# raviraina/grok

Measured on AMD Instinct MI355X. Metric: Mpixels/s encode+decode, 8K RGB 5/3 lossless + 9/7 lossy, 1/2/4/8 GPU, higher is better.
Workload: dtype int32 (5/3) + f32 (9/7)

## Files before the change

### grok_amd/csrc/gk_engine.cpp

```cpp
#include <hip/hip_runtime.h>

#include <algorithm>
#include <array>
#include <tuple>
#include <cmath>
#include <cstdarg>
#include <cstdlib>
#include <cstdio>
#include <cstring>
#include <memory>
#include <string>
#include <atomic>
#include <chrono>
#include <condition_variable>
#include <functional>
#include <mutex>
#include <thread>
#include <unordered_map>
#include <vector>
#include <queue>
#include <map>
#include <climits>
#include <linux/futex.h>
#include <sys/syscall.h>
// ... 2892 lines not shown
    bool dwt_partial = false;
    uint32_t dec_reduce = 0;
    bool win_whole_tile = false;
    int device = 0;
    bool registered = false;
    hipStream_t st = nullptr;
    hipStream_t aux[3] = {nullptr, nullptr, nullptr};
    hipEvent_t xev[6];
    std::string err;
    gk_timings tm{};
    std::string plan_key;
    Plan plan;
    DevBuf arena;
    DevBuf bytes;
    DevBuf dblocks;
    DevBuf dpasses;
    DevBuf dinfo;
    DevBuf dseg;
    DevBuf dout;
    DevBuf dplanes;
    DevBuf derr;
    DevBuf dsym, dsymoff, dpassend, dcminfo;
    DevBuf dmsstate, dseglen;
    DevBuf dscratch, dnmse, dord, dweight, dord_enc;
    HostBuf hinfo, hseg, hhdr, hpasses, hord, hweight, hord_enc;
    DevBuf dstage1, dstage2;
    DevBuf dcol_src, dcol_out, dcol_tab;
    DevBuf dpix_src, dpix_out;
    DevBuf dicc_tab;
    std::vector<uint8_t> icc_blob;
    DevBuf dpix_in;
    HostBuf hstage1, hstage2;
    int16_t* nmse_tab = nullptr;
    hipEvent_t ev[32];
    bool blocks_uploaded = false;
    uint32_t enc_b0 = 0, enc_b1 = 0;
    std::vector<uint8_t> enc_dx, enc_dy;
    EncColour enc_col;
    std::vector<uint8_t> enc_jp2h;
    std::vector<uint32_t> hdr_dx, hdr_dy, hdr_prec, hdr_sgnd;
    bool enc_rc = false;
    std::vector<std::pair<uint32_t, uint32_t>> native_qcd, band_qcd;
    std::vector<gk_band_result> rb_bands;
    std::vector<gk_block_result> rb_blocks;
    std::vector<gk_pass_result> rb_passes;
    std::vector<uint8_t> rb_data;
};

// ... 482 lines not shown
        ctx->blocks_uploaded = true; ctx->enc_b0 = b0; ctx->enc_b1 = b1; ctx->enc_rc = do_rc;
    }
    HIPCHK(hipMemsetAsync(derr, 0, 64, st));
    const uint32_t nsolo_env = []() { const char* v = getenv("GK_T1ENC_SOLO"); return v ? (uint32_t)atoi(v) : 0u; }();
    if (P.p.ht()) {
        uint8_t* mel = (uint8_t*)ctx->dsym.get((size_t)nbx * GK_HT_MEL_CAP + 256);
        launch_check(__LINE__);
        HIPCHK(hipEventRecord(ctx->ev[8], st));
        gk_launch_ht_enc(st, arena, dblk, dbytes, mel, GK_HT_MEL_CAP, dinfo, nbr, derr, P.p.wide());
    } else if (P.p.t1_generic()) {
        uint8_t* mst = (uint8_t*)ctx->dmsstate.get(gk_t1ms_state_bytes(nbx));
        launch_check(__LINE__);
        HIPCHK(hipEventRecord(ctx->ev[8], st));
        gk_launch_t1_enc_ms(st, arena, dblk, dbytes, dps, dinfo, nbr, derr, ctx->nmse_tab, dpcount, mst, P.p.cblk_sty & 0x3f);
    } else if (nbr < 8192 || getenv("GK_T1ENC_SERIAL")) {
        gk_launch_t1_cm(st, arena, dblk, dsymoff, dsym, dpe, dcm, nbr, derr, ctx->nmse_tab, dnmse);
        launch_check(__LINE__);
        HIPCHK(hipEventRecord(ctx->ev[8], st));
        gk_launch_t1_mq(st, dsym, dsymoff, dpe, dcm, dblk, dbytes, dps, dinfo, nbr, derr, dnmse, dpcount, nullptr, 0,
                        0xffffffffu, std::min(nsolo_env, nbr));
    } else {
        uint32_t* dw = (uint32_t*)ctx->dweight.get(4 * (size_t)nbr);
        gk_launch_t1_weight(st, arena, dblk, dw, nbr);
        uint32_t* hw = (uint32_t*)ctx->hweight.get(4 * (size_t)nbr);
        HIPCHK(hipMemcpyAsync(hw, dw, 4 * (size_t)nbr, hipMemcpyDeviceToHost, st));
        HIPCHK(hipStreamSynchronize(st));
        uint32_t wmax = 1;
        for (uint32_t i = 0; i < nbr; ++i) wmax = std::max(wmax, hw[i]);
        const uint32_t kB = 4096;
        auto key = [&](uint32_t i) { return kB - 1 - (uint32_t)(((uint64_t)hw[i] * (kB - 1)) / wmax); };
        std::vector<uint32_t> start(kB + 1, 0);
        for (uint32_t i = 0; i < nbr; ++i) start[key(i)]++;
        for (uint32_t k = 0, acc = 0; k <= kB; ++k) { const uint32_t c = start[k]; start[k] = acc; acc += c; }
        uint32_t* ho = (uint32_t*)ctx->hord_enc.get(4 * (size_t)nbr);
        for (uint32_t i = 0; i < nbr; ++i) ho[start[key(i)]++] = i;
        uint32_t* dord = (uint32_t*)ctx->dord_enc.get(4 * (size_t)nbr);
        HIPCHK(hipMemcpyAsync(dord, ho, 4 * (size_t)nbr, hipMemcpyHostToDevice, st));
        static std::vector<double> frs[2];
        std::vector<double>& fr = frs[do_rc ? 1 : 0];
        if (fr.empty()) {
            const char* cv = getenv("GK_T1ENC_CUTS");
            std::string cs = cv ? cv : (do_rc ? "0.08,0.25" : "0.125,0.375");
            for (size_t q = 0; q < cs.size();) {
                size_t e = cs.find(',', q);
                if (e == std::string::npos) e = cs.size();
                const double f = atof(cs.substr(q, e - q).c_str());
                if (f > 0 && f < 1 && fr.size() < 3) fr.push_back(f);
                q = e + 1;
            }
        }
        std::vector<uint32_t> cut(1, 0);
        for (double f : fr) {
            const uint32_t c = (uint32_t)(nbr * f) / 256 * 256;
            if (c > cut.back() && c < nbr) cut.push_back(c);
        }
        cut.push_back(nbr);
        const int nch = (int)cut.size() - 1;
        for (int k = 0; k < nch; ++k) {
            const uint32_t base = cut[k], cnt = cut[k + 1] - cut[k];
            gk_launch_t1_cm(st, arena, dblk, dsymoff, dsym, dpe, dcm, nbr, derr, ctx->nmse_tab, dnmse, dord, base, cnt);
// ... 1 lines not shown
                HIPCHK(hipEventRecord(ctx->xev[k], st));
                HIPCHK(hipStreamWaitEvent(ctx->aux[k], ctx->xev[k], 0));
                gk_launch_t1_mq(ctx->aux[k], dsym, dsymoff, dpe, dcm, dblk, dbytes, dps, dinfo, nbr, derr, dnmse, dpcount,
                                dord, base, cnt, k == 0 ? std::min(nsolo_env, cnt) : 0u);
                HIPCHK(hipEventRecord(ctx->xev[3 + k], ctx->aux[k]));
            } else {
                launch_check(__LINE__);
                HIPCHK(hipEventRecord(ctx->ev[8], st));
                gk_launch_t1_mq(st, dsym, dsymoff, dpe, dcm, dblk, dbytes, dps, dinfo, nbr, derr, dnmse, dpcount, dord,
                                base, cnt);
            }
        }
        for (int k = 0; k + 1 < nch; ++k) HIPCHK(hipStreamWaitEvent(st, ctx->xev[3 + k], 0));
    }
    launch_check(__LINE__);
    HIPCHK(hipEventRecord(ctx->ev[4], st));
    static const bool eprof = getenv("GK_PROFILE") != nullptr;
    using eclk = std::chrono::steady_clock;
    auto ems = [](eclk::time_point a, eclk::time_point b) { return std::chrono::duration<double, std::milli>(b - a).count(); };
    const auto te0 = eclk::now();
    uint32_t* hinfo = (uint32_t*)ctx->hinfo.get(16 * (size_t)nb + 64);
    HIPCHK(hipMemcpyAsync(hinfo + 4 * (size_t)b0, dinfo, 16 * (size_t)nbr, hipMemcpyDeviceToHost, st));
    HIPCHK(hipMemcpyAsync(hinfo + 4 * (size_t)nb, derr, 32, hipMemcpyDeviceToHost, st));
    HIPCHK(hipStreamSynchronize(st));
    const uint32_t t1err = hinfo[4 * (size_t)nb], npass_total = hinfo[4 * (size_t)nb + 4];
    if (t1err) throw GkError(t1err & 2 ? "T1 symbol buffer overflow" : "T1 code-block slot overflow");
    const bool ht = P.p.ht();
    const GkPass* hpasses = nullptr;
    if ((do_rc || (P.p.cblk_sty & (GK_STY_LAZY | GK_STY_TERMALL))) && !ht) {
        GkPass* hp = (GkPass*)ctx->hpasses.get(sizeof(GkPass) * (size_t)std::max(npass_total, 1u));
        HIPCHK(hipMemcpyAsync(hp, dps, sizeof(GkPass) * (size_t)npass_total, hipMemcpyDeviceToHost, st));
        HIPCHK(hipStreamSynchronize(st));
        hpasses = hp;
    }
    if (blocks_only) {
        dump_blocks(ctx, hinfo, dps, npass_total, dbytes, slot0);
        *rc = 0;
        return 0;
    }

    std::vector<uint8_t> H;
    H.reserve(1 << 12);
    size_t tlm_pos = 0;
    write_main_header(H, P, &tlm_pos);
    const size_t rc_header_size = H.size() + (P.p.jp2 ? jp2_prefix_size(P, ctx->enc_jp2h) : 0);
    if (!with_header) H.clear();
    const auto te1 = eclk::now();
    if (const char* ds = getenv("GK_DUMP_SYMS"); ds && dsym && !P.p.t1_generic()) {
        std::vector<uint32_t> pe((size_t)GK_MAX_PASSES * nbr), cm(2 * (size_t)nbr), out(2 * (size_t)nbr);
        HIPCHK(hipMemcpy(pe.data(), dpe, 4 * pe.size(), hipMemcpyDeviceToHost));
        HIPCHK(hipMemcpy(cm.data(), dcm, 4 * cm.size(), hipMemcpyDeviceToHost));
        for (uint32_t i = 0; i < nbr; ++i) {
            out[2 * i] = cm[2 * i + 1] ? pe[(size_t)GK_MAX_PASSES * i + cm[2 * i + 1] - 1] : 0;
            out[2 * i + 1] = cm[2 * i];
        }
        if (FILE* f = fopen(ds, "wb")) { fwrite(out.data(), 4, out.size(), f); fclose(f); }
    }
    if (const char* dp = getenv("GK_DUMP_PASSES")) {
        if (FILE* f = fopen(dp, "wb")) {
            const uint32_t hdr[2] = {nb, npass_total};
            fwrite(hdr, 4, 2, f);
            fwrite(hinfo, 16, nb, f);
            if (hpasses) fwrite(hpasses, sizeof(GkPass), npass_total, f);
            fclose(f);
        }
    }
    T2Enc T2(P, hinfo, hpasses, tb, te);
    std::vector<T2Enc::Swallow> tsw(te - tb);
    if (te - tb == 1 || !P.p.rate_control()) {
        T2.allocate(rc_header_size);
        tsw[0] = T2.final_sw;
    } else {
        const bool par = te - tb >= host_pool().size();
        auto one = [&](size_t q) {
            const uint32_t t = tb + (uint32_t)q;
            T2Enc Tt(P, hinfo, hpasses, t, t + 1);
            Tt.serial = par;
            Tt.allocate(rc_header_size);
            tsw[q] = Tt.final_sw;
            const TileG& TG = P.tiles[t];
            std::copy(Tt.lnp.begin() + (size_t)TG.b0 * T2.L, Tt.lnp.begin() + (size_t)TG.b1 * T2.L,
                      T2.lnp.begin() + (size_t)TG.b0 * T2.L);
        };
        if (par) host_pool().run(te - tb, one);
        else for (uint32_t q = 0; q < te - tb; ++q) one(q);
    }
    const auto te2 = eclk::now();
    std::vector<uint64_t> seg;
    seg.reserve(3 * ((size_t)nb * (ht ? 2 : 1) + 64));
    std::vector<uint8_t> hdrs;
// ... 250 lines not shown
                    if (ms) { seg.push_back(so); seg.push_back(pos); seg.push_back(ms); pos += ms; }
                    seg.push_back(so + G.data_cap - tl); seg.push_back(pos); seg.push_back(tl);
                    pos += tl;
                    continue;
                }
                seg.push_back(so + off); seg.push_back(pos); seg.push_back(n);
                pos += n;
            }
        }
        }
    }
    uint8_t eoc[2] = {0xff, 0xd9};
    if (with_header) add_host(eoc, 2);
    const size_t total = pos;
    if (jp2) {
        const size_t prefix = J.size();
        J.clear();
        write_jp2_prefix(J, P, total - prefix, ctx->enc_jp2h);
        memcpy(hdrs.data(), J.data(), J.size());
    }
    launch_check(__LINE__);
    HIPCHK(hipEventRecord(ctx->ev[5], st));
    if (eprof)
        fprintf(stderr, "encode t2: fetch %.2f ms, allocate %.2f ms, packets %.2f ms, segments %.2f ms\n", ems(te0, te1),
                ems(te1, te2), ems(te2, te3), ems(te3, eclk::now()));
    if (total > cap) { *rc = -2; return total; }
    if (hdrs.size() > (64u << 20)) throw GkError("packet headers exceed staging");
    uint8_t* hh = (uint8_t*)ctx->hhdr.get(hdrs.size());
    memcpy(hh, hdrs.data(), hdrs.size());
    HIPCHK(hipMemcpyAsync(dbytes + slot_span, hh, hdrs.size(), hipMemcpyHostToDevice, st));
    uint64_t* hs = (uint64_t*)ctx->hseg.get(seg.size() * 8);
    memcpy(hs, seg.data(), seg.size() * 8);
    uint64_t* ds = (uint64_t*)ctx->dseg.get(seg.size() * 8);
    HIPCHK(hipMemcpyAsync(ds, hs, seg.size() * 8, hipMemcpyHostToDevice, st));
    uint8_t* dst = out_on_device ? out : (uint8_t*)ctx->dout.get(total);
    gk_launch_gather(st, dbytes, dst, ds, (uint32_t)(seg.size() / 3));
    launch_check(__LINE__);
    HIPCHK(hipEventRecord(ctx->ev[6], st));
    if (!out_on_device) HIPCHK(hipMemcpyAsync(out, dst, total, hipMemcpyDeviceToHost, st));
    launch_check(__LINE__);
    HIPCHK(hipEventRecord(ctx->ev[7], st));
    HIPCHK(hipStreamSynchronize(st));
    ctx->tm.mct_ms = ev_ms(ctx, 1, 2);
    ctx->tm.dwt_ms = ev_ms(ctx, 2, 3);
    ctx->tm.t1_ms = ev_ms(ctx, 3, 4);
    ctx->tm.t1_cm_ms = ev_ms(ctx, 3, 8);
    ctx->tm.t1_coder_ms = ev_ms(ctx, 8, 4);
    ctx->tm.cs_bytes = total;
// ... 877 lines not shown
            }
            uint8_t* stage = (uint8_t*)ctx->dpix_out.get(tot);
            for (uint32_t k = 0; k < nout; ++k) { dst[k] = stage; stage += pitch[k] * sh[D.ch[k].from]; }
        } else {
            for (uint32_t k = 0; k < nout; ++k) { dst[k] = (uint8_t*)comps[k]; pitch[k] = (size_t)strides[k] * es_out; }
        }
        for (uint32_t k = 0; k < nout; ++k) {
            GkPixArgs a{};
            a.ch[0] = chan(k);
            a.w = sw[D.ch[k].from]; a.h = sh[D.ch[k].from]; a.nch = 1;
            a.dst = dst[k]; a.row_bytes = pitch[k];
            gk_launch_pixels(st, stype, dtype, a);
        }
        launch_check(__LINE__);
        HIPCHK(hipEventRecord(ctx->ev[23], st));
        if (!out_on_device)
            for (uint32_t k = 0; k < nout; ++k)
                HIPCHK(hipMemcpy2DAsync(comps[k], (size_t)strides[k] * es_out, dst[k], pitch[k], (size_t)sw[D.ch[k].from] * es_out,
                                        sh[D.ch[k].from], hipMemcpyDeviceToHost, st));
    }
    HIPCHK(hipStreamSynchronize(st));
    const float ms = ev_ms(ctx, 22, 23);
    ctx->tm.mct_ms += ms; ctx->tm.total_ms += ms;
}
static void decode_impl(gk_ctx* ctx, const uint8_t* cs, size_t len, int cs_on_device, void* const* comps,
                        const uint32_t* strides, uint32_t sample_bytes, int out_on_device, const uint32_t* win = nullptr,
                        const TilePass* pass = nullptr) {
    hipStream_t st = ctx->st;
    launch_check(__LINE__);
    HIPCHK(hipEventRecord(ctx->ev[0], st));
    const uint8_t* const cs_in = cs;
    const size_t len_in = len;
    ctx->dwt_partial = pass ? pass->partial : win != nullptr && !ctx->win_whole_tile;
    static const bool prof = getenv("GK_PROFILE") != nullptr;
    auto now = [] { return std::chrono::steady_clock::now(); };
    auto ms = [](std::chrono::steady_clock::time_point a, std::chrono::steady_clock::time_point b) {
        return std::chrono::duration<double, std::milli>(b - a).count();
    };
    const auto h0 = now();
    ByteSrc S;
    S.len = len; S.st = st;
    if (cs_on_device) S.dev = cs; else S.host = cs;
    Jp2Colour col;
    {
        size_t joff = 0, jlen = 0;
        const bool colour = (ctx->dec_colour || ctx->dec_display || !ctx->dec_prec.empty() || ctx->pix) && !ctx->col_inner && !pass;
// ... 578 lines not shown
            HIPCHK(hipMemsetAsync(derr, 0, 64, st));
            gk_launch_ht_dec(st, src_bytes, dblk, dsel, arena, nbr, derr, cls_wide);
            launch_check(__LINE__);
            HIPCHK(hipEventRecord(ctx->ev[8], st));
            int herr = 0;
            HIPCHK(hipMemcpyAsync(&herr, derr, 4, hipMemcpyDeviceToHost, st));
            HIPCHK(hipStreamSynchronize(st));
            if (herr) throw GkError("corrupt HT code-block segment");
        } else if (cls_generic) {
            uint32_t* dsl = nullptr;
            if ((cls_sty & (GK_STY_LAZY | GK_STY_TERMALL)) && !hseglen.empty()) {
                uint32_t* hsl = (uint32_t*)ctx->hord.get(4 * hseglen.size());
                memcpy(hsl, hseglen.data(), 4 * hseglen.size());
                dsl = (uint32_t*)ctx->dseglen.get(4 * hseglen.size());
                HIPCHK(hipMemcpyAsync(dsl, hsl, 4 * hseglen.size(), hipMemcpyHostToDevice, st));
            }
            uint8_t* mst = (uint8_t*)ctx->dmsstate.get(gk_t1ms_state_bytes(nbx));
            gk_launch_t1_dec_ms(st, src_bytes, dblk, dsl, arena, nbr, mst, cls_sty);
            launch_check(__LINE__);
            HIPCHK(hipEventRecord(ctx->ev[8], st));
            if (dsl) HIPCHK(hipStreamSynchronize(st));
        } else {
            const uint32_t L = gk_t1dec_lanes();
            GkSoloPlan sp = nbr ? gk_t1dec_solo_plan(nbr, L) : GkSoloPlan{0, -1, 1.f};
            const bool shared = sp.forced < 0 && engines_busy(ctx->device) > 1;
            uint32_t nsb = 0;
            std::vector<uint32_t> byl;
            std::vector<std::vector<uint32_t>> bins;
            auto weight = [&](uint32_t q) -> uint64_t { return blk[q].npasses ? blk[q].len : 0; };
            if (sp.waves) {
                const uint32_t kmax = sp.forced >= 0 ? (uint32_t)sp.forced : std::min<uint32_t>(nbr / 4, 4u * sp.waves);
                byl.resize(nbr);
                for (uint32_t q = 0; q < nbr; ++q) byl[q] = q;
                auto heavier = [&](uint32_t x, uint32_t y) { return weight(x) != weight(y) ? weight(x) > weight(y) : x < y; };
                const uint32_t top = std::min<uint32_t>(kmax + 1, nbr);
                if (top) {
                    std::nth_element(byl.begin(), byl.begin() + (top - 1), byl.end(), heavier);
                    std::sort(byl.begin(), byl.begin() + top, heavier);
                }
                auto pack = [&](uint32_t k, std::vector<std::vector<uint32_t>>* out) -> uint64_t {
                    std::vector<uint64_t> load(sp.waves, 0);
                    std::vector<uint32_t> cnt(sp.waves, 0);
                    if (out) out->assign(sp.waves, {});
                    using E = std::pair<uint64_t, uint32_t>;
                    std::priority_queue<E, std::vector<E>, std::greater<E>> pq;
                    for (uint32_t b = 0; b < sp.waves; ++b) pq.push({0, b});
                    uint64_t mx = 0;
                    for (uint32_t j = 0; j < k && !pq.empty(); ++j) {
                        const E e = pq.top();
                        pq.pop();
                        load[e.second] = e.first + weight(byl[j]);
                        mx = std::max(mx, load[e.second]);
                        if (out) (*out)[e.second].push_back(byl[j]);
                        if (++cnt[e.second] < 64) pq.push({load[e.second], e.second});
                    }
                    return mx;
                };
                uint32_t k = 0;
                if (sp.forced >= 0) {
                    k = (uint32_t)sp.forced;
                    bins.assign(sp.waves, {});
                    for (uint32_t j = 0; j < k; ++j) bins[j].push_back(byl[j]);
                } else if (shared) {
                    const uint32_t r = std::min<uint32_t>(std::max<uint32_t>(1024u, top), nbr - 1);
                    if (r >= top) std::nth_element(byl.begin() + top, byl.begin() + r, byl.end(), heavier);
                    const double ref = 1.3 * (double)weight(byl[r]);
                    while (k < std::min<uint32_t>(kmax, sp.waves) && (double)weight(byl[k]) > ref) ++k;
                    bins.assign(sp.waves, {});
                    for (uint32_t j = 0; j < k; ++j) bins[j].push_back(byl[j]);
                } else {
                    auto lane_side = [&](uint32_t kk) -> double { return kk < nbr ? (double)weight(byl[kk]) : 0.0; };
                    auto solo_side = [&](uint32_t kk) -> double { return (double)pack(kk, nullptr) / sp.ratio; };
                    uint32_t lo = 0, hi = kmax;
                    while (lo < hi) {
                        const uint32_t mid = (lo + hi) / 2;
                        if (solo_side(mid) >= lane_side(mid)) hi = mid; else lo = mid + 1;
                    }
                    k = lo;
                    if (k > 0 && std::max(solo_side(k - 1), lane_side(k - 1)) <= std::max(solo_side(k), lane_side(k))) --k;
                    if (k) pack(k, &bins);
                }
                nsb = k;
            }
            uint32_t nsw = 0;
            for (uint32_t b = 0; b < bins.size(); ++b)
                if (!bins[b].empty()) nsw = b + 1;
            nsw = (nsw + 11) / 12 * 12;
            const uint32_t nw = nsw + (nbr - nsb + L - 1) / L, nslots = nw * 64;
            uint32_t* hord = (uint32_t*)ctx->hord.get(4 * ((size_t)nslots + 2 * (size_t)nbr + 2) + 8 * ((size_t)nw + 1));
            uint32_t* hpos = hord + nslots;
            uint32_t* hids = hpos + nbr;
            uint64_t* hwo = (uint64_t*)(hids + nbr + 2);
            {
                std::fill(hord, hord + nslots, 0xffffffffu);
                std::vector<uint8_t> solo(nbr, 0);
                for (uint32_t b = 0; b < bins.size() && b < nsw; ++b)
                    for (uint32_t i = 0; i < bins[b].size(); ++i) {
                        const uint32_t q = bins[b][i];
                        solo[q] = 1;
                        hord[(size_t)b * 64 + i] = q; hpos[q] = b * 64 + i;
                    }
                std::vector<uint32_t> cnt(GK_MAX_PASSES + 2, 0);
                for (uint32_t q = 0; q < nbr; ++q)
                    if (!solo[q]) cnt[std::min<uint32_t>(blk[q].npasses, GK_MAX_PASSES + 1)]++;
                std::vector<uint32_t> start(GK_MAX_PASSES + 2, 0);
                uint32_t acc = 0;
                for (int k = GK_MAX_PASSES + 1; k >= 0; --k) { start[k] = acc; acc += cnt[k]; }
                for (uint32_t q = 0; q < nbr; ++q) {
                    hids[q] = q;
                    if (solo[q]) continue;
                    const uint32_t k = std::min<uint32_t>(blk[q].npasses, GK_MAX_PASSES + 1);
                    const uint32_t idx = start[k]++;
                    const uint32_t slot = (nsw + idx / L) * 64 + idx % L;
                    hord[slot] = q; hpos[q] = slot;
                }
                uint64_t wo = 0;
                for (uint32_t wv = 0; wv < nw; ++wv) {
                    hwo[wv] = wo;
                    uint32_t mp = 0;
                    for (uint32_t i = wv * 64; i < wv * 64 + (wv < nsw ? 64 : L); ++i)
                        if (hord[i] != 0xffffffffu) mp = std::max(mp, (uint32_t)blk[hord[i]].numbps);
                    if (wv < nsw && hord[wv * 64] == 0xffffffffu) continue;
                    wo += (272 + (uint64_t)mp * 64) * 64;
                }
                hwo[nw] = wo;
            }
            const size_t obytes = 4 * ((size_t)nslots + 2 * (size_t)nbr + 2) + 8 * ((size_t)nw + 1);
            uint32_t* dord = (uint32_t*)ctx->dord.get(obytes);
            HIPCHK(hipMemcpyAsync(dord, hord, obytes, hipMemcpyHostToDevice, st));
            const uint32_t* dpos = dord + nslots;
            const uint32_t* dids = dpos + nbr;
            const uint64_t* dwo = (const uint64_t*)(dids + nbr + 2);
            uint64_t* dscr = (uint64_t*)ctx->dscratch.get(8 * hwo[nw] + 64);
            HIPCHK(hipMemsetAsync(dscr + hwo[nsw], 0, 8 * (hwo[nw] - hwo[nsw]), st));
            gk_launch_t1_dec(st, src_bytes, dblk, dord, dscr, dwo, nslots, nsw);
            ctx->tm.t1_steps_max = ctx->tm.t1_steps_total = ctx->tm.t1_symbols = 0;
            ctx->tm.t1_solo_decisions = ctx->tm.t1_solo_decisions_max = 0;
            ctx->tm.t1_solo_blocks = nsb;
            ctx->tm.t1_shared += (shared && sp.waves) ? 1 : 0;
            if (getenv("GK_T1_STATS")) {
                uint64_t sv[5];
                gk_t1dec_stats(sv);
                ctx->tm.t1_steps_max = sv[0]; ctx->tm.t1_steps_total = sv[1]; ctx->tm.t1_symbols = sv[2];
                ctx->tm.t1_solo_decisions = sv[3]; ctx->tm.t1_solo_decisions_max = sv[4];
            }
            launch_check(__LINE__);
            HIPCHK(hipEventRecord(ctx->ev[8], st));
            uint32_t maxnp = 1;
            for (uint32_t q = 0; q < nbr; ++q) maxnp = std::max<uint32_t>(maxnp, blk[q].numbps);
            gk_launch_t1_recon(st, dblk, dids, dpos, dscr, dwo, arena, nbr, maxnp);
        }
    };
    for (size_t k = 0; k < cls_range.size(); ++k) {
        const uint32_t s0 = cls_range[k].first, e0 = k + 1 < cls_range.size() ? cls_range[k + 1].first : nbr;
        if (k) HIPCHK(hipStreamSynchronize(st));
        t1_class(s0, e0 - s0, cls_range[k].second);
    }
    launch_check(__LINE__);
    HIPCHK(hipEventRecord(ctx->ev[3], st));
    std::vector<int32_t> shiftv(P.nc), mnv(P.nc), mxv(P.nc);
    for (uint32_t c = 0; c < P.nc; ++c) {
        const uint32_t pr = P.c_prec(c);
        const bool sg = P.c_sgnd(c) != 0;
        shiftv[c] = sg ? 0 : (1 << (pr - 1));
        mnv[c] = sg ? -(1 << (pr - 1)) : 0;
        mxv[c] = sg ? (1 << (pr - 1)) - 1 : (int32_t)((1u << pr) - 1);
        if ((sample_bytes == 1 || sample_bytes == 2) && sg != (P.sgnd != 0))
            throw GkError("8 / 16-bit output of components with different signs: use int32 planes");
    }
    const int stype = sample_type(sample_bytes, P.prec, P.sgnd != 0);
    const size_t es = gk_sample_size(stype);
    const bool mct3r = P.mct3();
    if (red) {
// ... 802 lines not shown
```

### grok_amd/csrc/gk_launch.h

```cpp
#pragma once
#include <hip/hip_runtime.h>
#include <stdint.h>
#include "gk_common.h"

#define GK_SAMPLE_DISPATCH(t, T, ...)                            \
    switch (t) {                                                 \
        case GK_U8: { typedef uint8_t T; __VA_ARGS__; break; }   \
        case GK_S8: { typedef int8_t T; __VA_ARGS__; break; }    \
        case GK_U16: { typedef uint16_t T; __VA_ARGS__; break; } \
        case GK_S16: { typedef int16_t T; __VA_ARGS__; break; }  \
        default: { typedef int32_t T; __VA_ARGS__; break; }      \
    }

void gk_launch_dc_rct_fwd(hipStream_t st, int stype, const void* r, const void* g, const void* b, uint32_t sin,
                          int32_t* y, int32_t* u, int32_t* v, uint32_t sout, uint32_t w, uint32_t h, int32_t shift);
void gk_launch_dc_fwd(hipStream_t st, int stype, const void* in, uint32_t sin, int32_t* out, uint32_t sout, uint32_t w,
                      uint32_t h, int32_t shift);
void gk_launch_rct_inv_dc(hipStream_t st, const int32_t* y, const int32_t* u, const int32_t* v, uint32_t sin, int stype,
                          void* r, void* g, void* b, uint32_t sout, uint32_t w, uint32_t h, int32_t shift,
                          int32_t mn, int32_t mx);
void gk_launch_dc_inv(hipStream_t st, const int32_t* in, uint32_t sin, int stype, void* out, uint32_t sout, uint32_t w,
                      uint32_t h, int32_t shift, int32_t mn, int32_t mx);
uint32_t gk_dwt_cpw(uint32_t wgs, uint32_t n, bool multi);
void gk_launch_dwt53_fwd(hipStream_t st, const int32_t* src, uint32_t sstride, int32_t* dst, uint32_t dstride,
                         uint32_t w, uint32_t h, GkTiles tb = GkTiles(), GkComps cs = GkComps());
void gk_launch_dwt53_inv(hipStream_t st, const int32_t* src, uint32_t sstride, int32_t* dst, uint32_t dstride,
                         uint32_t w, uint32_t h, GkTiles tb = GkTiles(), GkComps cs = GkComps());
void gk_launch_dwt53_fwd_l1(hipStream_t st, int stype, int nc, GkPtr3 in, uint32_t sin, int32_t* dst, uint64_t cstride,
                            uint32_t dstride, uint32_t w, uint32_t h, GkTiles tb, int32_t shift);
void gk_launch_dwt53_inv_l1(hipStream_t st, int stype, int nc, const int32_t* src, uint64_t cstride, uint32_t sstride,
                            GkPtr3 out, uint32_t ostride, GkWin win, uint32_t w, uint32_t h, GkTiles tb, int32_t shift,
                            int32_t mn, int32_t mx);
void gk_launch_gather(hipStream_t st, const uint8_t* src, uint8_t* dst, const uint64_t* seg, uint32_t nseg);
void gk_launch_t1_cm(hipStream_t st, const int32_t* coef, const GkBlock* blocks, const uint64_t* sym_off, uint8_t* sym,
                     uint32_t* pass_end, uint32_t* cm_info, uint32_t nblocks, int* err, const int16_t* nmse_tab,
                     int32_t* pass_nmse, const uint32_t* order = nullptr, uint32_t base = 0, uint32_t count = 0xffffffffu);
void gk_launch_t1_mq(hipStream_t st, const uint8_t* sym, const uint64_t* sym_off, const uint32_t* pass_end,
                     const uint32_t* cm_info, const GkBlock* blocks, uint8_t* bytes, GkPass* passes, uint32_t* info,
                     uint32_t nblocks, int* err, const int32_t* pass_nmse, uint32_t* pass_counter,
                     const uint32_t* order = nullptr, uint32_t base = 0, uint32_t count = 0xffffffffu,
                     uint32_t nsolo = 0);
void gk_launch_t1_weight(hipStream_t st, const int32_t* coef, const GkBlock* blocks, uint32_t* weight, uint32_t nblocks);
uint32_t gk_t1dec_lanes();
void gk_t1dec_stats(uint64_t out[5]);
struct GkSoloPlan { uint32_t waves; int forced; float ratio; };
GkSoloPlan gk_t1dec_solo_plan(uint32_t nblocks, uint32_t lanes);
void gk_launch_t1_dec(hipStream_t st, const uint8_t* bytes, const GkBlock* blocks, const uint32_t* order,
                      uint64_t* scratch, const uint64_t* wave_off, uint32_t nblocks, uint32_t nsolo);
void gk_launch_t1_recon(hipStream_t st, const GkBlock* blocks, const uint32_t* ids, const uint32_t* pos,
                        const uint64_t* scratch, const uint64_t* wave_off, int32_t* coef, uint32_t nblocks,
                        uint32_t maxnp);
void gk_launch_dwt_any(hipStream_t st, bool irrev, bool forward, int32_t* in, int32_t* out, uint32_t stride, uint32_t w,
                       uint32_t h, uint32_t px, uint32_t py, GkTiles tb, GkComps cs, bool partial = false);
void gk_launch_t1_enc_ms(hipStream_t st, const int32_t* coef, const GkBlock* blocks, uint8_t* bytes, GkPass* passes,
                         uint32_t* info, uint32_t nblocks, int* err, const int16_t* nmse_tab, uint32_t* pass_counter,
                         uint8_t* state, uint32_t sty);
void gk_launch_t1_dec_ms(hipStream_t st, const uint8_t* bytes, const GkBlock* blocks, const uint32_t* seglen, int32_t* coef,
                         uint32_t nblocks, uint8_t* state, uint32_t sty);
size_t gk_t1ms_state_bytes(uint32_t nblocks);
void gk_launch_dc_ict_fwd(hipStream_t st, int stype, const void* r, const void* g, const void* b, uint32_t sin, float* y,
                          float* u, float* v, uint32_t sout, uint32_t w, uint32_t h, int32_t shift);
void gk_launch_dc_fwd_f(hipStream_t st, int stype, const void* in, uint32_t sin, float* out, uint32_t sout, uint32_t w,
                        uint32_t h, int32_t shift);
void gk_launch_ict_inv_dc(hipStream_t st, const float* y, const float* u, const float* v, uint32_t sin, int stype, void* r,
                          void* g, void* b, uint32_t sout, uint32_t w, uint32_t h, int32_t shift, int32_t mn,
// ... 140 lines not shown
```

### grok_amd/csrc/gk_t1enc.hip

```cpp
#include <hip/hip_runtime.h>
#include <stdint.h>
#include "gk_common.h"
#include "gk_t1_common.h"
#include <algorithm>
#include <type_traits>
#include <cstdlib>

#define SYM_PER_PLANE 11264u

__device__ __forceinline__ uint32_t win6(uint64_t col, uint32_t s) {
    return (uint32_t)((s ? (col >> (4 * s - 1)) : (col << 1)) & 63u);
}

__device__ __forceinline__ uint32_t lane_prev(uint32_t v) {
    return (uint32_t)__builtin_amdgcn_update_dpp(0, (int)v, 0x138, 0xf, 0xf, false);
}
__device__ __forceinline__ uint32_t lane_next(uint32_t v) {
    return (uint32_t)__builtin_amdgcn_update_dpp(0, (int)v, 0x130, 0xf, 0xf, false);
}
__device__ __forceinline__ uint32_t wave_excl_scan(uint32_t v, uint32_t& total) {
    int inc = (int)v;
    inc += __builtin_amdgcn_update_dpp(0, inc, 0x111, 0xf, 0xf, false);
    inc += __builtin_amdgcn_update_dpp(0, inc, 0x112, 0xf, 0xf, false);
    inc += __builtin_amdgcn_update_dpp(0, inc, 0x114, 0xf, 0xf, false);
// ... 691 lines not shown
            const int32_t raw = coef[B.band_off + (size_t)y * B.stride + lane];
            const uint32_t a0 = irrev ? (uint32_t)fabsf(rintf((__int_as_float(raw) / B.step) * 64.0f))
                                      : (uint32_t)(raw < 0 ? -raw : raw) * 64u;
            const uint32_t a = ((a0 >> 6) << (6 + (B.flags >> 3))) | (a0 & 63u);
            mx = a > mx ? a : mx;
            nbits += (a >> 6) ? 32u - __clz(a >> 6) : 0u;
        }
#pragma unroll
    for (int o = 32; o > 0; o >>= 1) {
        const uint32_t t = __shfl_xor(mx, o); mx = t > mx ? t : mx;
        nbits += __shfl_xor(nbits, o);
    }
    if (lane == 0) {
        const uint32_t t = mx ? 32 - __clz(mx) : 0;
        const uint32_t planes = t <= 6 ? 0 : t - 6;
        const uint32_t rows = (B.h + 3) / 4;
        weight[b] = planes * B.w * B.h * 5u + (uint32_t)((3ull * nbits * B.h) / (rows ? rows : 1));
    }
}
void gk_launch_t1_weight(hipStream_t st, const int32_t* coef, const GkBlock* blocks, uint32_t* weight, uint32_t nblocks) {
    if (!nblocks) return;
    hipLaunchKernelGGL(k_t1_weight, dim3(nblocks), dim3(64), 0, st, coef, blocks, weight, nblocks);
}
void gk_launch_t1_mq(hipStream_t st, const uint8_t* sym, const uint64_t* sym_off, const uint32_t* pass_end,
                     const uint32_t* cm_info, const GkBlock* blocks, uint8_t* bytes, GkPass* passes, uint32_t* info,
                     uint32_t nblocks, int* err, const int32_t* pass_nmse, uint32_t* pass_counter, const uint32_t* order,
                     uint32_t base, uint32_t count, uint32_t nsolo) {
    if (!nblocks) return;
    if (count == 0xffffffffu) count = nblocks;
    if (!count) return;
    nsolo = std::min((nsolo + 3) / 4 * 4, (count + 3) / 4 * 4);
    static const uint32_t nl = [] {
        const char* v = getenv("GK_T1ENC_LANES");
        const int n = v ? atoi(v) : 64;
        return (uint32_t)(n < 1 ? 1 : (n > 64 ? 64 : n));
    }();
    const size_t pe = (size_t)(GK_MAX_PASSES + 1) * nl * 4 * 4;
    const size_t lds = std::max(pe, (size_t)163840 - 4 * sizeof(MqLds));
    const uint32_t rest = count > nsolo ? count - nsolo : 0;
    hipLaunchKernelGGL(k_t1_mq, dim3(nsolo / 4 + (rest + 4 * nl - 1) / (4 * nl)), dim3(256), lds, st, sym, sym_off,
                       pass_end, cm_info, blocks, bytes, passes, info, nblocks, err, pass_nmse, pass_counter, nl, order,
                       base, count, nsolo);
}
```

Before: 1748.

## Sort T1 encode block order on GPU and overlap T2 setup with T1

Replaces the host-side bucket sort of code-block weights, which needed a device-to-host copy and a stream sync, with a GPU max reduction, key kernel and rocPRIM radix sort, so the encoder no longer stalls before launching the MQ coder. T2 encoder state is now constructed before waiting on the T1 results so it overlaps GPU work. The decoder solo-plan construction is refactored to sort packed 64-bit keys and to compute the greedy packing once instead of repeatedly inside the binary search. It adds rocPRIM temp storage and extra kernel launches, and the order must match the previous stable bucket sort.

After: 1748. About the same (-0.0%).

```diff
diff --git a/grok_amd/csrc/gk_engine.cpp b/grok_amd/csrc/gk_engine.cpp
--- a/grok_amd/csrc/gk_engine.cpp
+++ b/grok_amd/csrc/gk_engine.cpp
@@ -2938,8 +2938,8 @@
     DevBuf derr;
     DevBuf dsym, dsymoff, dpassend, dcminfo;
     DevBuf dmsstate, dseglen;
-    DevBuf dscratch, dnmse, dord, dweight, dord_enc;
-    HostBuf hinfo, hseg, hhdr, hpasses, hord, hweight, hord_enc;
+    DevBuf dscratch, dnmse, dord, dweight, dord_enc, dorder_tmp;
+    HostBuf hinfo, hseg, hhdr, hpasses, hord;
     DevBuf dstage1, dstage2;
     DevBuf dcol_src, dcol_out, dcol_tab;
     DevBuf dpix_src, dpix_out;
@@ -3468,20 +3468,9 @@
     } else {
         uint32_t* dw = (uint32_t*)ctx->dweight.get(4 * (size_t)nbr);
         gk_launch_t1_weight(st, arena, dblk, dw, nbr);
-        uint32_t* hw = (uint32_t*)ctx->hweight.get(4 * (size_t)nbr);
-        HIPCHK(hipMemcpyAsync(hw, dw, 4 * (size_t)nbr, hipMemcpyDeviceToHost, st));
-        HIPCHK(hipStreamSynchronize(st));
-        uint32_t wmax = 1;
-        for (uint32_t i = 0; i < nbr; ++i) wmax = std::max(wmax, hw[i]);
-        const uint32_t kB = 4096;
-        auto key = [&](uint32_t i) { return kB - 1 - (uint32_t)(((uint64_t)hw[i] * (kB - 1)) / wmax); };
-        std::vector<uint32_t> start(kB + 1, 0);
-        for (uint32_t i = 0; i < nbr; ++i) start[key(i)]++;
-        for (uint32_t k = 0, acc = 0; k <= kB; ++k) { const uint32_t c = start[k]; start[k] = acc; acc += c; }
-        uint32_t* ho = (uint32_t*)ctx->hord_enc.get(4 * (size_t)nbr);
-        for (uint32_t i = 0; i < nbr; ++i) ho[start[key(i)]++] = i;
         uint32_t* dord = (uint32_t*)ctx->dord_enc.get(4 * (size_t)nbr);
-        HIPCHK(hipMemcpyAsync(dord, ho, 4 * (size_t)nbr, hipMemcpyHostToDevice, st));
+        const size_t obytes = gk_t1_order_bytes(nbr);
+        HIPCHK(gk_launch_t1_order(st, dw, dord, nbr, ctx->dorder_tmp.get(obytes), obytes));
         static std::vector<double> frs[2];
         std::vector<double>& fr = frs[do_rc ? 1 : 0];
         if (fr.empty()) {
@@ -3529,7 +3518,11 @@
     uint32_t* hinfo = (uint32_t*)ctx->hinfo.get(16 * (size_t)nb + 64);
     HIPCHK(hipMemcpyAsync(hinfo + 4 * (size_t)b0, dinfo, 16 * (size_t)nbr, hipMemcpyDeviceToHost, st));
     HIPCHK(hipMemcpyAsync(hinfo + 4 * (size_t)nb, derr, 32, hipMemcpyDeviceToHost, st));
+    std::unique_ptr<T2Enc> T2p;
+    if (!blocks_only) T2p.reset(new T2Enc(P, hinfo, nullptr, tb, te));
+    const auto te0a = eclk::now();
     HIPCHK(hipStreamSynchronize(st));
+    const auto te0b = eclk::now();
     const uint32_t t1err = hinfo[4 * (size_t)nb], npass_total = hinfo[4 * (size_t)nb + 4];
     if (t1err) throw GkError(t1err & 2 ? "T1 symbol buffer overflow" : "T1 code-block slot overflow");
     const bool ht = P.p.ht();
@@ -3572,7 +3565,8 @@
             fclose(f);
         }
     }
-    T2Enc T2(P, hinfo, hpasses, tb, te);
+    T2Enc& T2 = *T2p;
+    T2.passes = hpasses;
     std::vector<T2Enc::Swallow> tsw(te - tb);
     if (te - tb == 1 || !P.p.rate_control()) {
         T2.allocate(rc_header_size);
@@ -3869,8 +3863,9 @@
     launch_check(__LINE__);
     HIPCHK(hipEventRecord(ctx->ev[5], st));
     if (eprof)
-        fprintf(stderr, "encode t2: fetch %.2f ms, allocate %.2f ms, packets %.2f ms, segments %.2f ms\n", ems(te0, te1),
-                ems(te1, te2), ems(te2, te3), ems(te3, eclk::now()));
+        fprintf(stderr, "encode t2: fetch %.2f ms (T2 state %.2f ms beside T1, wait for T1 %.2f ms, pass records + header %.2f ms), "
+                        "allocate %.2f ms, packets %.2f ms, segments %.2f ms\n",
+                ems(te0, te1), ems(te0, te0a), ems(te0a, te0b), ems(te0b, te1), ems(te1, te2), ems(te2, te3), ems(te3, eclk::now()));
     if (total > cap) { *rc = -2; return total; }
     if (hdrs.size() > (64u << 20)) throw GkError("packet headers exceed staging");
     uint8_t* hh = (uint8_t*)ctx->hhdr.get(hdrs.size());
@@ -4794,6 +4789,127 @@
     HIPCHK(hipStreamSynchronize(st));
     const float ms = ev_ms(ctx, 22, 23);
     ctx->tm.mct_ms += ms; ctx->tm.total_ms += ms;
+}
+struct T1DecPlan { uint32_t nsb = 0, nsw = 0, nw = 0, nslots = 0, maxnp = 1; };
+static uint32_t t1dec_plan_nwmax(uint32_t nbr, uint32_t L, const GkSoloPlan& sp) {
+    return (sp.waves + 11) / 12 * 12 + (nbr + L - 1) / L;
+}
+static size_t t1dec_plan_words(uint32_t nbr, uint32_t nwmax, uint32_t nslots) {
+    return 2 * (size_t)nbr + 2 + 2 * ((size_t)nwmax + 1) + nslots;
+}
+static T1DecPlan t1dec_plan(const GkBlock* blk, uint32_t nbr, uint32_t L, const GkSoloPlan& sp, bool shared, uint32_t* tab,
+                            uint32_t nwmax) {
+    T1DecPlan R;
+    uint32_t nsb = 0;
+    std::vector<std::vector<uint32_t>> bins;
+    if (sp.waves) {
+        std::vector<uint64_t> keys(nbr);
+        for (uint32_t q = 0; q < nbr; ++q)
+            keys[q] = ((uint64_t)(blk[q].npasses ? blk[q].len : 0) << 32) | (0xffffffffu - q);
+        auto kw = [&](uint32_t j) -> uint64_t { return keys[j] >> 32; };
+        auto kq = [&](uint32_t j) -> uint32_t { return 0xffffffffu - (uint32_t)keys[j]; };
+        const uint32_t kmax = sp.forced >= 0 ? (uint32_t)sp.forced : std::min<uint32_t>(nbr / 4, 4u * sp.waves);
+        const uint32_t top = std::min<uint32_t>(kmax + 1, nbr);
+        if (top) {
+            std::nth_element(keys.begin(), keys.begin() + (top - 1), keys.end(), std::greater<uint64_t>());
+            std::sort(keys.begin(), keys.begin() + top, std::greater<uint64_t>());
+        }
+        uint32_t k = 0;
+        if (sp.forced >= 0) {
+            k = (uint32_t)sp.forced;
+            bins.assign(sp.waves, {});
+            for (uint32_t j = 0; j < k; ++j) bins[j].push_back(kq(j));
+        } else if (shared) {
+            const uint32_t r = std::min<uint32_t>(std::max<uint32_t>(1024u, top), nbr - 1);
+            if (r >= top) std::nth_element(keys.begin() + top, keys.begin() + r, keys.end(), std::greater<uint64_t>());
+            const double ref = 1.3 * (double)kw(r);
+            while (k < std::min<uint32_t>(kmax, sp.waves) && (double)kw(k) > ref) ++k;
+            bins.assign(sp.waves, {});
+            for (uint32_t j = 0; j < k; ++j) bins[j].push_back(kq(j));
+        } else {
+            std::vector<uint64_t> load(sp.waves, 0), mxload(kmax + 1, 0);
+            std::vector<uint32_t> cnt(sp.waves, 0), wave_of(kmax, 0xffffffffu);
+            {
+                using E = std::pair<uint64_t, uint32_t>;
+                std::priority_queue<E, std::vector<E>, std::greater<E>> pq;
+                for (uint32_t b = 0; b < sp.waves; ++b) pq.push({0, b});
+                uint64_t mx = 0;
+                for (uint32_t j = 0; j < kmax; ++j) {
+                    if (!pq.empty()) {
+                        const E e = pq.top();
+                        pq.pop();
+                        load[e.second] = e.first + kw(j);
+                        mx = std::max(mx, load[e.second]);
+                        wave_of[j] = e.second;
+                        if (++cnt[e.second] < 64) pq.push({load[e.second], e.second});
+                    }
+                    mxload[j + 1] = mx;
+                }
+            }
+            auto lane_side = [&](uint32_t kk) -> double { return kk < nbr ? (double)kw(kk) : 0.0; };
+            auto solo_side = [&](uint32_t kk) -> double { return (double)mxload[kk] / sp.ratio; };
+            uint32_t lo = 0, hi = kmax;
+            while (lo < hi) {
+                const uint32_t mid = (lo + hi) / 2;
+                if (solo_side(mid) >= lane_side(mid)) hi = mid; else lo = mid + 1;
+            }
+            k = lo;
+            if (k > 0 && std::max(solo_side(k - 1), lane_side(k - 1)) <= std::max(solo_side(k), lane_side(k))) --k;
+            if (k) {
+                bins.assign(sp.waves, {});
+                for (uint32_t j = 0; j < k; ++j)
+                    if (wave_of[j] != 0xffffffffu) bins[wave_of[j]].push_back(kq(j));
+            }
+        }
+        nsb = k;
+    }
+    uint32_t nsw = 0;
+    for (uint32_t b = 0; b < bins.size(); ++b)
+        if (!bins[b].empty()) nsw = b + 1;
+    nsw = (nsw + 11) / 12 * 12;
+    const uint32_t nw = nsw + (nbr - nsb + L - 1) / L, nslots = nw * 64;
+    if (nw > nwmax) throw GkError("internal: T1 decoder plan larger than its table");
+    uint32_t* hpos = tab;
+    uint32_t* hids = hpos + nbr;
+    uint64_t* hwo = (uint64_t*)(hids + nbr + 2);
+    uint32_t* hord = (uint32_t*)(hwo + nwmax + 1);
+    std::fill(hord, hord + nslots, 0xffffffffu);
+    std::vector<uint8_t> solo(nbr, 0);
+    for (uint32_t b = 0; b < bins.size() && b < nsw; ++b)
+        for (uint32_t i = 0; i < bins[b].size(); ++i) {
+            const uint32_t q = bins[b][i];
+            solo[q] = 1;
+            hord[(size_t)b * 64 + i] = q; hpos[q] = b * 64 + i;
+        }
+    std::vector<uint32_t> cnt(GK_MAX_PASSES + 2, 0);
+    uint32_t maxnp = 1;
+    for (uint32_t q = 0; q < nbr; ++q) {
+        maxnp = std::max<uint32_t>(maxnp, blk[q].numbps);
+        if (!solo[q]) cnt[std::min<uint32_t>(blk[q].npasses, GK_MAX_PASSES + 1)]++;
+    }
+    std::vector<uint32_t> start(GK_MAX_PASSES + 2, 0);
+    uint32_t acc = 0;
+    for (int k = GK_MAX_PASSES + 1; k >= 0; --k) { start[k] = acc; acc += cnt[k]; }
+    for (uint32_t q = 0; q < nbr; ++q) {
+        hids[q] = q;
+        if (solo[q]) continue;
+        const uint32_t k = std::min<uint32_t>(blk[q].npasses, GK_MAX_PASSES + 1);
+        const uint32_t idx = start[k]++;
+        const uint32_t slot = (nsw + idx / L) * 64 + idx % L;
+        hord[slot] = q; hpos[q] = slot;
+    }
+    uint64_t wo = 0;
+    for (uint32_t wv = 0; wv < nw; ++wv) {
+        hwo[wv] = wo;
+        uint32_t mp = 0;
+        for (uint32_t i = wv * 64; i < wv * 64 + (wv < nsw ? 64 : L); ++i)
+            if (hord[i] != 0xffffffffu) mp = std::max(mp, (uint32_t)blk[hord[i]].numbps);
+        if (wv < nsw && hord[wv * 64] == 0xffffffffu) continue;
+        wo += (272 + (uint64_t)mp * 64) * 64;
+    }
+    hwo[nw] = wo;
+    R.nsb = nsb; R.nsw = nsw; R.nw = nw; R.nslots = nslots; R.maxnp = maxnp;
+    return R;
 }
 static void decode_impl(gk_ctx* ctx, const uint8_t* cs, size_t len, int cs_on_device, void* const* comps,
                         const uint32_t* strides, uint32_t sample_bytes, int out_on_device, const uint32_t* win = nullptr,
@@ -5418,115 +5534,20 @@
             if (dsl) HIPCHK(hipStreamSynchronize(st));
         } else {
             const uint32_t L = gk_t1dec_lanes();
-            GkSoloPlan sp = nbr ? gk_t1dec_solo_plan(nbr, L) : GkSoloPlan{0, -1, 1.f};
+            const GkSoloPlan sp = gk_t1dec_solo_plan(nbr, L);
             const bool shared = sp.forced < 0 && engines_busy(ctx->device) > 1;
-            uint32_t nsb = 0;
-            std::vector<uint32_t> byl;
-            std::vector<std::vector<uint32_t>> bins;
-            auto weight = [&](uint32_t q) -> uint64_t { return blk[q].npasses ? blk[q].len : 0; };
-            if (sp.waves) {
-                const uint32_t kmax = sp.forced >= 0 ? (uint32_t)sp.forced : std::min<uint32_t>(nbr / 4, 4u * sp.waves);
-                byl.resize(nbr);
-                for (uint32_t q = 0; q < nbr; ++q) byl[q] = q;
-                auto heavier = [&](uint32_t x, uint32_t y) { return weight(x) != weight(y) ? weight(x) > weight(y) : x < y; };
-                const uint32_t top = std::min<uint32_t>(kmax + 1, nbr);
-                if (top) {
-                    std::nth_element(byl.begin(), byl.begin() + (top - 1), byl.end(), heavier);
-                    std::sort(byl.begin(), byl.begin() + top, heavier);
-                }
-                auto pack = [&](uint32_t k, std::vector<std::vector<uint32_t>>* out) -> uint64_t {
-                    std::vector<uint64_t> load(sp.waves, 0);
-                    std::vector<uint32_t> cnt(sp.waves, 0);
-                    if (out) out->assign(sp.waves, {});
-                    using E = std::pair<uint64_t, uint32_t>;
-                    std::priority_queue<E, std::vector<E>, std::greater<E>> pq;
-                    for (uint32_t b = 0; b < sp.waves; ++b) pq.push({0, b});
-                    uint64_t mx = 0;
-                    for (uint32_t j = 0; j < k && !pq.empty(); ++j) {
-                        const E e = pq.top();
-                        pq.pop();
-                        load[e.second] = e.first + weight(byl[j]);
-                        mx = std::max(mx, load[e.second]);
-                        if (out) (*out)[e.second].push_back(byl[j]);
-                        if (++cnt[e.second] < 64) pq.push({load[e.second], e.second});
-                    }
-                    return mx;
-                };
-                uint32_t k = 0;
-                if (sp.forced >= 0) {
-                    k = (uint32_t)sp.forced;
-                    bins.assign(sp.waves, {});
-                    for (uint32_t j = 0; j < k; ++j) bins[j].push_back(byl[j]);
-                } else if (shared) {
-                    const uint32_t r = std::min<uint32_t>(std::max<uint32_t>(1024u, top), nbr - 1);
-                    if (r >= top) std::nth_element(byl.begin() + top, byl.begin() + r, byl.end(), heavier);
-                    const double ref = 1.3 * (double)weight(byl[r]);
-                    while (k < std::min<uint32_t>(kmax, sp.waves) && (double)weight(byl[k]) > ref) ++k;
-                    bins.assign(sp.waves, {});
-                    for (uint32_t j = 0; j < k; ++j) bins[j].push_back(byl[j]);
-                } else {
-                    auto lane_side = [&](uint32_t kk) -> double { return kk < nbr ? (double)weight(byl[kk]) : 0.0; };
-                    auto solo_side = [&](uint32_t kk) -> double { return (double)pack(kk, nullptr) / sp.ratio; };
-                    uint32_t lo = 0, hi = kmax;
-                    while (lo < hi) {
-                        const uint32_t mid = (lo + hi) / 2;
-                        if (solo_side(mid) >= lane_side(mid)) hi = mid; else lo = mid + 1;
-                    }
-                    k = lo;
-                    if (k > 0 && std::max(solo_side(k - 1), lane_side(k - 1)) <= std::max(solo_side(k), lane_side(k))) --k;
-                    if (k) pack(k, &bins);
-                }
-                nsb = k;
-            }
-            uint32_t nsw = 0;
-            for (uint32_t b = 0; b < bins.size(); ++b)
-                if (!bins[b].empty()) nsw = b + 1;
-            nsw = (nsw + 11) / 12 * 12;
-            const uint32_t nw = nsw + (nbr - nsb + L - 1) / L, nslots = nw * 64;
-            uint32_t* hord = (uint32_t*)ctx->hord.get(4 * ((size_t)nslots + 2 * (size_t)nbr + 2) + 8 * ((size_t)nw + 1));
-            uint32_t* hpos = hord + nslots;
-            uint32_t* hids = hpos + nbr;
-            uint64_t* hwo = (uint64_t*)(hids + nbr + 2);
-            {
-                std::fill(hord, hord + nslots, 0xffffffffu);
-                std::vector<uint8_t> solo(nbr, 0);
-                for (uint32_t b = 0; b < bins.size() && b < nsw; ++b)
-                    for (uint32_t i = 0; i < bins[b].size(); ++i) {
-                        const uint32_t q = bins[b][i];
-                        solo[q] = 1;
-                        hord[(size_t)b * 64 + i] = q; hpos[q] = b * 64 + i;
-                    }
-                std::vector<uint32_t> cnt(GK_MAX_PASSES + 2, 0);
-                for (uint32_t q = 0; q < nbr; ++q)
-                    if (!solo[q]) cnt[std::min<uint32_t>(blk[q].npasses, GK_MAX_PASSES + 1)]++;
-                std::vector<uint32_t> start(GK_MAX_PASSES + 2, 0);
-                uint32_t acc = 0;
-                for (int k = GK_MAX_PASSES + 1; k >= 0; --k) { start[k] = acc; acc += cnt[k]; }
-                for (uint32_t q = 0; q < nbr; ++q) {
-                    hids[q] = q;
-                    if (solo[q]) continue;
-                    const uint32_t k = std::min<uint32_t>(blk[q].npasses, GK_MAX_PASSES + 1);
-                    const uint32_t idx = start[k]++;
-                    const uint32_t slot = (nsw + idx / L) * 64 + idx % L;
-                    hord[slot] = q; hpos[q] = slot;
-                }
-                uint64_t wo = 0;
-                for (uint32_t wv = 0; wv < nw; ++wv) {
-                    hwo[wv] = wo;
-                    uint32_t mp = 0;
-                    for (uint32_t i = wv * 64; i < wv * 64 + (wv < nsw ? 64 : L); ++i)
-                        if (hord[i] != 0xffffffffu) mp = std::max(mp, (uint32_t)blk[hord[i]].numbps);
-                    if (wv < nsw && hord[wv * 64] == 0xffffffffu) continue;
-                    wo += (272 + (uint64_t)mp * 64) * 64;
-                }
-                hwo[nw] = wo;
-            }
-            const size_t obytes = 4 * ((size_t)nslots + 2 * (size_t)nbr + 2) + 8 * ((size_t)nw + 1);
-            uint32_t* dord = (uint32_t*)ctx->dord.get(obytes);
-            HIPCHK(hipMemcpyAsync(dord, hord, obytes, hipMemcpyHostToDevice, st));
-            const uint32_t* dpos = dord + nslots;
+            const uint32_t nwmax = t1dec_plan_nwmax(nbr, L, sp);
+            uint32_t* const tab = (uint32_t*)ctx->hord.get(4 * t1dec_plan_words(nbr, nwmax, nwmax * 64));
+            const T1DecPlan tp = t1dec_plan(blk, nbr, L, sp, shared, tab, nwmax);
+            const uint32_t nsb = tp.nsb, nsw = tp.nsw, nw = tp.nw, nslots = tp.nslots;
+            const uint64_t* hwo = (const uint64_t*)(tab + 2 * (size_t)nbr + 2);
+            const size_t obytes = 4 * t1dec_plan_words(nbr, nwmax, nslots);
+            uint32_t* dtab = (uint32_t*)ctx->dord.get(obytes);
+            HIPCHK(hipMemcpyAsync(dtab, tab, obytes, hipMemcpyHostToDevice, st));
+            const uint32_t* dpos = dtab;
             const uint32_t* dids = dpos + nbr;
             const uint64_t* dwo = (const uint64_t*)(dids + nbr + 2);
+            const uint32_t* dord = (const uint32_t*)(dwo + nwmax + 1);
             uint64_t* dscr = (uint64_t*)ctx->dscratch.get(8 * hwo[nw] + 64);
             HIPCHK(hipMemsetAsync(dscr + hwo[nsw], 0, 8 * (hwo[nw] - hwo[nsw]), st));
             gk_launch_t1_dec(st, src_bytes, dblk, dord, dscr, dwo, nslots, nsw);
@@ -5542,9 +5563,7 @@
             }
             launch_check(__LINE__);
             HIPCHK(hipEventRecord(ctx->ev[8], st));
-            uint32_t maxnp = 1;
-            for (uint32_t q = 0; q < nbr; ++q) maxnp = std::max<uint32_t>(maxnp, blk[q].numbps);
-            gk_launch_t1_recon(st, dblk, dids, dpos, dscr, dwo, arena, nbr, maxnp);
+            gk_launch_t1_recon(st, dblk, dids, dpos, dscr, dwo, arena, nbr, tp.maxnp);
         }
     };
     for (size_t k = 0; k < cls_range.size(); ++k) {
diff --git a/grok_amd/csrc/gk_launch.h b/grok_amd/csrc/gk_launch.h
--- a/grok_amd/csrc/gk_launch.h
+++ b/grok_amd/csrc/gk_launch.h
@@ -41,6 +41,8 @@
                      const uint32_t* order = nullptr, uint32_t base = 0, uint32_t count = 0xffffffffu,
                      uint32_t nsolo = 0);
 void gk_launch_t1_weight(hipStream_t st, const int32_t* coef, const GkBlock* blocks, uint32_t* weight, uint32_t nblocks);
+size_t gk_t1_order_bytes(uint32_t nblocks);
+hipError_t gk_launch_t1_order(hipStream_t st, const uint32_t* weight, uint32_t* order, uint32_t nblocks, void* tmp, size_t tmp_bytes);
 uint32_t gk_t1dec_lanes();
 void gk_t1dec_stats(uint64_t out[5]);
 struct GkSoloPlan { uint32_t waves; int forced; float ratio; };
diff --git a/grok_amd/csrc/gk_t1enc.hip b/grok_amd/csrc/gk_t1enc.hip
--- a/grok_amd/csrc/gk_t1enc.hip
+++ b/grok_amd/csrc/gk_t1enc.hip
@@ -1,4 +1,5 @@
 #include <hip/hip_runtime.h>
+#include <rocprim/device/device_radix_sort.hpp>
 #include <stdint.h>
 #include "gk_common.h"
 #include "gk_t1_common.h"
@@ -737,6 +738,49 @@
     if (!nblocks) return;
     hipLaunchKernelGGL(k_t1_weight, dim3(nblocks), dim3(64), 0, st, coef, blocks, weight, nblocks);
 }
+
+static const uint32_t kOrderBuckets = 4096, kOrderBits = 12;
+__global__ __launch_bounds__(1024) void k_t1_wmax(const uint32_t* __restrict__ weight, uint32_t* __restrict__ wmax, uint32_t n) {
+    __shared__ uint32_t part[16];
+    uint32_t m = 0;
+    for (uint32_t i = threadIdx.x; i < n; i += 1024) m = max(m, weight[i]);
+#pragma unroll
+    for (int o = 32; o > 0; o >>= 1) m = max(m, (uint32_t)__shfl_xor(m, o));
+    if ((threadIdx.x & 63) == 0) part[threadIdx.x >> 6] = m;
+    __syncthreads();
+    if (threadIdx.x == 0) {
+        for (int k = 1; k < 16; ++k) m = max(m, part[k]);
+        *wmax = m ? m : 1u;
+    }
+}
+__global__ __launch_bounds__(256) void k_t1_okeys(const uint32_t* __restrict__ weight, const uint32_t* __restrict__ wmax,
+                                                  uint32_t* __restrict__ key, uint32_t* __restrict__ idx, uint32_t n) {
+    const uint32_t i = blockIdx.x * 256 + threadIdx.x;
+    if (i >= n) return;
+    key[i] = kOrderBuckets - 1 - (uint32_t)(((uint64_t)weight[i] * (kOrderBuckets - 1)) / *wmax);
+    idx[i] = i;
+}
+static size_t t1_order_sort_bytes(uint32_t n) {
+    size_t b = 0;
+    uint32_t* p = nullptr;
+    if (rocprim::radix_sort_pairs(nullptr, b, p, p, p, p, (size_t)n, 0u, kOrderBits, (hipStream_t) nullptr) != hipSuccess) return 0;
+    return b;
+}
+static size_t t1_order_head_bytes(uint32_t n) { return (16 + 3 * (size_t)n) * 4 + 256; }
+size_t gk_t1_order_bytes(uint32_t nblocks) { return t1_order_head_bytes(nblocks) + t1_order_sort_bytes(nblocks) + 256; }
+hipError_t gk_launch_t1_order(hipStream_t st, const uint32_t* weight, uint32_t* order, uint32_t nblocks, void* tmp, size_t tmp_bytes) {
+    if (!nblocks) return hipSuccess;
+    if (tmp_bytes < gk_t1_order_bytes(nblocks)) return hipErrorInvalidValue;
+    uint32_t* wmax = (uint32_t*)tmp;
+    uint32_t* kin = wmax + 16;
+    uint32_t* kout = kin + nblocks;
+    uint32_t* iin = kout + nblocks;
+    void* sort_tmp = (void*)(((uintptr_t)(iin + nblocks) + 255) & ~(uintptr_t)255);
+    size_t sort_bytes = t1_order_sort_bytes(nblocks);
+    hipLaunchKernelGGL(k_t1_wmax, dim3(1), dim3(1024), 0, st, weight, wmax, nblocks);
+    hipLaunchKernelGGL(k_t1_okeys, dim3((nblocks + 255) / 256), dim3(256), 0, st, weight, wmax, kin, iin, nblocks);
+    return rocprim::radix_sort_pairs(sort_tmp, sort_bytes, kin, kout, iin, order, (size_t)nblocks, 0u, kOrderBits, st);
+}
 void gk_launch_t1_mq(hipStream_t st, const uint8_t* sym, const uint64_t* sym_off, const uint32_t* pass_end,
                      const uint32_t* cm_info, const GkBlock* blocks, uint8_t* bytes, GkPass* passes, uint32_t* info,
                      uint32_t nblocks, int* err, const int32_t* pass_nmse, uint32_t* pass_counter, const uint32_t* order,
```
